# Z1HaoC/YOLO-Dual

Hardware: AMD Instinct MI355X
Metric: images/sec at 640x640 bs=16/GPU (higher is better)
Workload: dtype bf16; 1 GPU; YOLOv5-backbone (C3+SPPF) + UNet-lite SegmentHead, fwd+bwd+SGD/EMA step, 640x640, bs=16/GPU, CE+0.5*Dice, 12 classes (BASELINE configs[1]); global_batch=16, parallelism=dp1

## Files before the change

### yolo_dual_amd/csrc/spatial.hip

```cpp
#include "common.h"
#include <stdlib.h>

static inline int sgrid(long long total) {
    long long b = (total + 255) / 256;
    if (b > 256 * 16) b = 256 * 16;
    if (b < 1) b = 1;
    return (int)b;
}

template <typename T>
__global__ __launch_bounds__(256) void maxpool_fwd_kernel(const T* __restrict__ x, int ldx, T* __restrict__ y, int ldy,
                                                          uint8_t* __restrict__ idx, int N, int Hi, int Wi, int Ho, int Wo,
                                                          int Cp, int k, int s, int p) {
    constexpr int V = ET<T>::V;
    const int cpp = Cp / V;
    const long long total = (long long)N * Ho * Wo * cpp;
    for (long long i = (long long)blockIdx.x * blockDim.x + threadIdx.x; i < total; i += (long long)gridDim.x * blockDim.x) {
        int cq = (int)(i % cpp);
        long long pix = i / cpp;
        int wo = (int)(pix % Wo);
        long long t2 = pix / Wo;
        int ho = (int)(t2 % Ho);
        int n = (int)(t2 / Ho);
        float best[V];
        int bi[V];
#pragma unroll
        for (int e = 0; e < V; ++e) { best[e] = -INFINITY; bi[e] = 0; }
        bool first = true;
        for (int ky = 0; ky < k; ++ky) {
            int ih = ho * s - p + ky;
            if ((unsigned)ih >= (unsigned)Hi) continue;
            for (int kx = 0; kx < k; ++kx) {
                int iw = wo * s - p + kx;
                if ((unsigned)iw >= (unsigned)Wi) continue;
                float v[V];
                unpack16<T>(*(const uint4*)(x + ((size_t)(n * Hi + ih) * Wi + iw) * ldx + cq * V), v);
#pragma unroll
                for (int e = 0; e < V; ++e) {
                    if (first || v[e] > best[e] || v[e] != v[e]) { best[e] = v[e]; bi[e] = ky * k + kx; }
                }
                first = false;
            }
        }
        *(uint4*)(y + (size_t)pix * ldy + cq * V) = pack16<T>(best);
        if (idx) {
#pragma unroll
            for (int e = 0; e < V; ++e) idx[(size_t)pix * Cp + cq * V + e] = (uint8_t)bi[e];
        }
    }
}

template <typename T>
__global__ __launch_bounds__(256) void maxpool_bwd_kernel(const T* __restrict__ dy, int lddy, const uint8_t* __restrict__ idx,
                                                          T* __restrict__ dx, int lddx, int accumulate, int N, int Hi, int Wi,
                                                          int Ho, int Wo, int Cp, int k, int s, int p) {
    constexpr int V = ET<T>::V;
    const int cpp = Cp / V;
    const long long total = (long long)N * Hi * Wi * cpp;
    for (long long i = (long long)blockIdx.x * blockDim.x + threadIdx.x; i < total; i += (long long)gridDim.x * blockDim.x) {
        int cq = (int)(i % cpp);
        long long pix = i / cpp;
        int iw = (int)(pix % Wi);
        long long t2 = pix / Wi;
        int ih = (int)(t2 % Hi);
        int n = (int)(t2 / Hi);
        float g[V];
#pragma unroll
        for (int e = 0; e < V; ++e) g[e] = 0.f;
        if (accumulate) unpack16<T>(*(const uint4*)(dx + (size_t)pix * lddx + cq * V), g);
        for (int ky = 0; ky < k; ++ky) {
            int nh = ih + p - ky;
            if (nh < 0 || nh % s != 0) continue;
            int ho = nh / s;
            if (ho >= Ho) continue;
            for (int kx = 0; kx < k; ++kx) {
                int nw = iw + p - kx;
                if (nw < 0 || nw % s != 0) continue;
                int wo = nw / s;
                if (wo >= Wo) continue;
                size_t op = ((size_t)(n * Ho + ho) * Wo + wo);
                float d[V];
                unpack16<T>(*(const uint4*)(dy + op * lddy + cq * V), d);
                const uint8_t* ip = idx + op * Cp + cq * V;
                int code = ky * k + kx;
#pragma unroll
                for (int e = 0; e < V; ++e) g[e] += (ip[e] == code) ? d[e] : 0.f;
            }
        }
        *(uint4*)(dx + (size_t)pix * lddx + cq * V) = pack16<T>(g);
    }
}

extern "C" int ydl_maxpool_fwd(int dtype, const void* x, int ldx, void* y, int ldy, uint8_t* idx,
                               int N, int Hi, int Wi, int Ho, int Wo, int C, int k, int s, int p, void* stream) {
    const int V = dtype == YDL_F32 ? 4 : 8;
    const int Cp = round_up(C, V);
    YDL_CHECK(x && y && ldx >= Cp && ldy >= Cp && k * k <= 255, "bad arguments");
    YDL_CHECK(Ho == (Hi + 2 * p - k) / s + 1 && Wo == (Wi + 2 * p - k) / s + 1, "output size mismatch");
    hipStream_t st = (hipStream_t)stream;
    int grid = sgrid((long long)N * Ho * Wo * (Cp / V));
    if (dtype == YDL_F32) maxpool_fwd_kernel<float><<<grid, 256, 0, st>>>((const float*)x, ldx, (float*)y, ldy, idx, N, Hi, Wi, Ho, Wo, Cp, k, s, p);
    else maxpool_fwd_kernel<bf16_t><<<grid, 256, 0, st>>>((const bf16_t*)x, ldx, (bf16_t*)y, ldy, idx, N, Hi, Wi, Ho, Wo, Cp, k, s, p);
    YDL_LAUNCH_CHECK();
    return 0;
}
extern "C" int ydl_maxpool_bwd(int dtype, const void* dy, int lddy, const uint8_t* idx, void* dx, int lddx, int accumulate,
                               int N, int Hi, int Wi, int Ho, int Wo, int C, int k, int s, int p, void* stream) {
    const int V = dtype == YDL_F32 ? 4 : 8;
    const int Cp = round_up(C, V);
    YDL_CHECK(dy && dx && idx && lddy >= Cp && lddx >= Cp, "bad arguments");
    hipStream_t st = (hipStream_t)stream;
    int grid = sgrid((long long)N * Hi * Wi * (Cp / V));
    if (dtype == YDL_F32) maxpool_bwd_kernel<float><<<grid, 256, 0, st>>>((const float*)dy, lddy, idx, (float*)dx, lddx, accumulate, N, Hi, Wi, Ho, Wo, Cp, k, s, p);
    else maxpool_bwd_kernel<bf16_t><<<grid, 256, 0, st>>>((const bf16_t*)dy, lddy, idx, (bf16_t*)dx, lddx, accumulate, N, Hi, Wi, Ho, Wo, Cp, k, s, p);
    YDL_LAUNCH_CHECK();
    return 0;
}

template <int V> struct SpCodes;
template <> struct SpCodes<8> {
    typedef uint2 W;
    __device__ static __forceinline__ W pack(const int* c) {
        return make_uint2((unsigned)c[0] | ((unsigned)c[1] << 8) | ((unsigned)c[2] << 16) | ((unsigned)c[3] << 24),
                          (unsigned)c[4] | ((unsigned)c[5] << 8) | ((unsigned)c[6] << 16) | ((unsigned)c[7] << 24));
    }
    __device__ static __forceinline__ int get(const W& w, int e) { return (int)(((e < 4 ? w.x : w.y) >> ((e & 3) * 8)) & 0xffu); }
};
template <> struct SpCodes<4> {
    typedef unsigned W;
    __device__ static __forceinline__ W pack(const int* c) {
        return (unsigned)c[0] | ((unsigned)c[1] << 8) | ((unsigned)c[2] << 16) | ((unsigned)c[3] << 24);
    }
    __device__ static __forceinline__ int get(const W& w, int e) { return (int)((w >> (e * 8)) & 0xffu); }
};
#define SP_CG 2
template <typename T>
__global__ __launch_bounds__(256) void sppf_pool_fwd_kernel(const T* __restrict__ x, int ldx, T* __restrict__ y1, T* __restrict__ y2,
                                                            T* __restrict__ y3, int ldy, uint8_t* __restrict__ i1, uint8_t* __restrict__ i2,
                                                            uint8_t* __restrict__ i3, int H, int W, int Cp, int k) {
    constexpr int V = ET<T>::V;
    extern __shared__ __attribute__((aligned(16))) unsigned char sp_smem[];
    const int HW = H * W;
    const int items = HW * SP_CG;
    uint4* cur = (uint4*)sp_smem;
    uint4* rmax = cur + items;
    typedef SpCodes<V> CW;
    typename CW::W* rkx = (typename CW::W*)(rmax + items);
    const int cpp = Cp / V;
    const int n = blockIdx.y;
    const int cq0 = blockIdx.x * SP_CG;
    const int p = k / 2;
    for (int it = threadIdx.x; it < items; it += 256) {
        const int cg = it % SP_CG, pix = it / SP_CG;
        uint4 v = make_uint4(0, 0, 0, 0);
        if (cq0 + cg < cpp) v = *(const uint4*)(x + ((size_t)n * HW + pix) * ldx + (cq0 + cg) * V);
        cur[it] = v;
    }
    __syncthreads();
    T* const ys[3] = {y1, y2, y3};
    uint8_t* const is[3] = {i1, i2, i3};
#pragma unroll
    for (int st = 0; st < 3; ++st) {
        for (int it = threadIdx.x; it < items; it += 256) {
            const int cg = it % SP_CG, pix = it / SP_CG;
            const int wo = pix % W, ho = pix / W;
            float best[V];
            int bk[V];
#pragma unroll
            for (int e = 0; e < V; ++e) { best[e] = -INFINITY; bk[e] = 0; }
            bool first = true;
            for (int kx = 0; kx < k; ++kx) {
                const int iw = wo - p + kx;
                if ((unsigned)iw >= (unsigned)W) continue;
                float v[V];
                unpack16<T>(cur[(ho * W + iw) * SP_CG + cg], v);
#pragma unroll
                for (int e = 0; e < V; ++e)
                    if (first || v[e] > best[e] || v[e] != v[e]) { best[e] = v[e]; bk[e] = kx; }
                first = false;
            }
            rmax[it] = pack16<T>(best);
            rkx[it] = CW::pack(bk);
        }
        __syncthreads();
        for (int it = threadIdx.x; it < items; it += 256) {
            const int cg = it % SP_CG, pix = it / SP_CG;
            const int wo = pix % W, ho = pix / W;
            float best[V];
            int bi[V];
#pragma unroll
            for (int e = 0; e < V; ++e) { best[e] = -INFINITY; bi[e] = 0; }
            bool first = true;
            for (int ky = 0; ky < k; ++ky) {
                const int ih = ho - p + ky;
                if ((unsigned)ih >= (unsigned)H) continue;
                const int rit = (ih * W + wo) * SP_CG + cg;
                float v[V];
                unpack16<T>(rmax[rit], v);
                const typename CW::W rk = rkx[rit];
#pragma unroll
                for (int e = 0; e < V; ++e)
                    if (first || v[e] > best[e] || v[e] != v[e]) { best[e] = v[e]; bi[e] = ky * k + CW::get(rk, e); }
                first = false;
            }
            const uint4 o = pack16<T>(best);
            if (st < 2) cur[it] = o;
            if (cq0 + cg < cpp) {
                const size_t gp = (size_t)n * HW + pix;
                *(uint4*)(ys[st] + gp * ldy + (cq0 + cg) * V) = o;
                if (is[st]) *(typename CW::W*)(is[st] + gp * Cp + (cq0 + cg) * V) = CW::pack(bi);
            }
        }
        __syncthreads();
    }
}

template <typename T>
__global__ __launch_bounds__(256) void sppf_pool_bwd_kernel(const T* __restrict__ dy1, const T* __restrict__ dy2, const T* __restrict__ dy3,
                                                            int lddy, const uint8_t* __restrict__ i1, const uint8_t* __restrict__ i2,
                                                            const uint8_t* __restrict__ i3, T* __restrict__ dx, int lddx, int accumulate,
                                                            int H, int W, int Cp, int k) {
    constexpr int V = ET<T>::V;
    extern __shared__ __attribute__((aligned(16))) unsigned char sp_smem[];
    const int HW = H * W;
    uint4* plane[2] = {(uint4*)sp_smem, (uint4*)sp_smem + (size_t)HW * SP_CG};
    typedef SpCodes<V> CW;
    typename CW::W* icode = (typename CW::W*)((uint4*)sp_smem + (size_t)2 * HW * SP_CG);
    const int cpp = Cp / V;
    const int n = blockIdx.y;
    const int cq0 = blockIdx.x * SP_CG;
    const int p = k / 2;
    const int items = HW * SP_CG;
    const T* const dys[3] = {dy3, dy2, dy1};
    const uint8_t* const is[3] = {i3, i2, i1};
    for (int it = threadIdx.x; it < items; it += 256) {
        const int cg = it % SP_CG, pix = it / SP_CG;
        uint4 v = make_uint4(0, 0, 0, 0);
        if (cq0 + cg < cpp) v = *(const uint4*)(dy3 + ((size_t)n * HW + pix) * lddy + (cq0 + cg) * V);
        plane[0][it] = v;
    }
#pragma unroll
    for (int st = 0; st < 3; ++st) {
        for (int it = threadIdx.x; it < items; it += 256) {
            const int cg = it % SP_CG, pix = it / SP_CG;
            if (cq0 + cg < cpp) icode[it] = *(const typename CW::W*)(is[st] + ((size_t)n * HW + pix) * Cp + (cq0 + cg) * V);
        }
        __syncthreads();
        const uint4* src = plane[st & 1];
        uint4* dst = plane[(st + 1) & 1];
        for (int it = threadIdx.x; it < items; it += 256) {
            const int cg = it % SP_CG, pix = it / SP_CG;
            if (cq0 + cg >= cpp) continue;
            const int iw = pix % W, ih = pix / W;
            const size_t gp = (size_t)n * HW + pix;
            float g[V];
#pragma unroll
            for (int e = 0; e < V; ++e) g[e] = 0.f;
            if (st < 2) unpack16<T>(*(const uint4*)(dys[st + 1] + gp * lddy + (cq0 + cg) * V), g);
            else if (accumulate) unpack16<T>(*(const uint4*)(dx + gp * lddx + (cq0 + cg) * V), g);
            for (int ky = 0; ky < k; ++ky) {
                const int ho = ih + p - ky;
                if (ho < 0 || ho >= H) continue;
                for (int kx = 0; kx < k; ++kx) {
                    const int wo = iw + p - kx;
                    if (wo < 0 || wo >= W) continue;
                    const int oit = (ho * W + wo) * SP_CG + cg;
                    float d[V];
                    unpack16<T>(src[oit], d);
                    const typename CW::W cw = icode[oit];
                    const int code = ky * k + kx;
#pragma unroll
                    for (int e = 0; e < V; ++e) g[e] += (CW::get(cw, e) == code) ? d[e] : 0.f;
                }
            }
            const uint4 o = pack16<T>(g);
            if (st < 2) dst[it] = o;
            else *(uint4*)(dx + gp * lddx + (cq0 + cg) * V) = o;
        }
        __syncthreads();
    }
}

static inline size_t sppf_smem(int dtype, int H, int W, bool bwd) {
    const int V = dtype == YDL_F32 ? 4 : 8;
    (void)bwd;
    return (size_t)H * W * SP_CG * (2 * 16 + V);
}
extern "C" int ydl_sppf_pool_supported(int dtype, int H, int W, int C, int k) {
    if (dtype != YDL_F32 && dtype != YDL_BF16) return 0;
    if (k < 1 || k % 2 == 0 || k * k > 255 || H < 1 || W < 1 || C < 1) return 0;
    return sppf_smem(dtype, H, W, true) <= 64 * 1024 ? 1 : 0;
}
extern "C" int ydl_sppf_pool_fwd(int dtype, const void* x, int ldx, void* y1, void* y2, void* y3, int ldy,
                                 uint8_t* idx1, uint8_t* idx2, uint8_t* idx3, int N, int H, int W, int C, int k, void* stream) {
    const int V = dtype == YDL_F32 ? 4 : 8;
    const int Cp = round_up(C, V);
    YDL_CHECK(ydl_sppf_pool_supported(dtype, H, W, C, k), "plane too large for the LDS-resident form (query ydl_sppf_pool_supported)");
    YDL_CHECK(x && y1 && y2 && y3 && ldx >= Cp && ldy >= Cp && N >= 1, "bad arguments");
    YDL_CHECK((idx1 == nullptr) == (idx2 == nullptr) && (idx2 == nullptr) == (idx3 == nullptr), "the three index planes come together");
    YDL_CHECK(aligned16(x) && aligned16(y1) && aligned16(y2) && aligned16(y3) && ldx % V == 0 && ldy % V == 0, "16-byte alignment");
    hipStream_t st = (hipStream_t)stream;
    const dim3 grid((Cp / V + SP_CG - 1) / SP_CG, N);
    const size_t smem = sppf_smem(dtype, H, W, false);
    if (dtype == YDL_F32) sppf_pool_fwd_kernel<float><<<grid, 256, smem, st>>>((const float*)x, ldx, (float*)y1, (float*)y2, (float*)y3, ldy, idx1, idx2, idx3, H, W, Cp, k);
    else sppf_pool_fwd_kernel<bf16_t><<<grid, 256, smem, st>>>((const bf16_t*)x, ldx, (bf16_t*)y1, (bf16_t*)y2, (bf16_t*)y3, ldy, idx1, idx2, idx3, H, W, Cp, k);
    YDL_LAUNCH_CHECK();
    return 0;
}
extern "C" int ydl_sppf_pool_bwd(int dtype, const void* dy1, const void* dy2, const void* dy3, int lddy, const uint8_t* idx1,
                                 const uint8_t* idx2, const uint8_t* idx3, void* dx, int lddx, int accumulate,
                                 int N, int H, int W, int C, int k, void* stream) {
    const int V = dtype == YDL_F32 ? 4 : 8;
    const int Cp = round_up(C, V);
    YDL_CHECK(ydl_sppf_pool_supported(dtype, H, W, C, k), "plane too large for the LDS-resident form (query ydl_sppf_pool_supported)");
    YDL_CHECK(dy1 && dy2 && dy3 && idx1 && idx2 && idx3 && dx && lddy >= Cp && lddx >= Cp && N >= 1, "bad arguments");
    YDL_CHECK(aligned16(dy1) && aligned16(dy2) && aligned16(dy3) && aligned16(dx) && lddy % V == 0 && lddx % V == 0, "16-byte alignment");
    hipStream_t st = (hipStream_t)stream;
    const dim3 grid((Cp / V + SP_CG - 1) / SP_CG, N);
    const size_t smem = sppf_smem(dtype, H, W, true);
    if (dtype == YDL_F32) sppf_pool_bwd_kernel<float><<<grid, 256, smem, st>>>((const float*)dy1, (const float*)dy2, (const float*)dy3, lddy, idx1, idx2, idx3, (float*)dx, lddx, accumulate, H, W, Cp, k);
    else sppf_pool_bwd_kernel<bf16_t><<<grid, 256, smem, st>>>((const bf16_t*)dy1, (const bf16_t*)dy2, (const bf16_t*)dy3, lddy, idx1, idx2, idx3, (bf16_t*)dx, lddx, accumulate, H, W, Cp, k);
    YDL_LAUNCH_CHECK();
    return 0;
}

struct Lin { int i0, i1; float w0, w1; };

__device__ __forceinline__ Lin lin_src(int dst, float scale, int in, bool align) {
    Lin L;
    float src;
    if (align) {
        src = __fmul_rn(scale, (float)dst);
    } else {
        src = __fsub_rn(__fmul_rn(scale, __fadd_rn((float)dst, 0.5f)), 0.5f);
        if (src < 0.f) src = 0.f;
    }
    L.i0 = (int)src;
    if (L.i0 > in - 1) L.i0 = in - 1;
    L.i1 = L.i0 + (L.i0 < in - 1 ? 1 : 0);
    L.w1 = __fsub_rn(src, (float)L.i0);
    L.w0 = __fsub_rn(1.f, L.w1);
    return L;
}
__device__ __forceinline__ int near_src(int dst, float scale, int in) {
    int v = (int)floorf(__fmul_rn((float)dst, scale));
    return v < in - 1 ? v : in - 1;
}

template <typename T>
__global__ __launch_bounds__(256) void resize_fwd_kernel(int mode, const T* __restrict__ x, int ldx, T* __restrict__ y, int ldy,
                                                         int N, int Hi, int Wi, int Ho, int Wo, int Cp, float sh, float sw) {
    constexpr int V = ET<T>::V;
    const int cpp = Cp / V;
    const long long total = (long long)N * Ho * Wo * cpp;
    for (long long i = (long long)blockIdx.x * blockDim.x + threadIdx.x; i < total; i += (long long)gridDim.x * blockDim.x) {
        int cq = (int)(i % cpp);
        long long pix = i / cpp;
        int wo = (int)(pix % Wo);
        long long t2 = pix / Wo;
        int ho = (int)(t2 % Ho);
        int n = (int)(t2 / Ho);
        const T* xb = x + (size_t)n * Hi * Wi * ldx + cq * V;
        float o[V];
        if (mode == 0) {
            int ih = near_src(ho, sh, Hi), iw = near_src(wo, sw, Wi);
            *(uint4*)(y + (size_t)pix * ldy + cq * V) = *(const uint4*)(xb + ((size_t)ih * Wi + iw) * ldx);
            continue;
        }
        Lin lh = lin_src(ho, sh, Hi, mode == 2), lw = lin_src(wo, sw, Wi, mode == 2);
        float v00[V], v01[V], v10[V], v11[V];
        unpack16<T>(*(const uint4*)(xb + ((size_t)lh.i0 * Wi + lw.i0) * ldx), v00);
        unpack16<T>(*(const uint4*)(xb + ((size_t)lh.i0 * Wi + lw.i1) * ldx), v01);
        unpack16<T>(*(const uint4*)(xb + ((size_t)lh.i1 * Wi + lw.i0) * ldx), v10);
        unpack16<T>(*(const uint4*)(xb + ((size_t)lh.i1 * Wi + lw.i1) * ldx), v11);
#pragma unroll
        for (int e = 0; e < V; ++e)
            o[e] = lh.w0 * (lw.w0 * v00[e] + lw.w1 * v01[e]) + lh.w1 * (lw.w0 * v10[e] + lw.w1 * v11[e]);
        *(uint4*)(y + (size_t)pix * ldy + cq * V) = pack16<T>(o);
    }
}

__device__ __forceinline__ void cand_range(int i, int in, int out, float scale, int mode, int& lo, int& hi) {
    float inv = scale > 0.f ? 1.0f / scale : (float)out;
    float a = ((float)i - 1.5f) * inv - 2.f, b = ((float)i + 1.5f) * inv + 2.f;
    if (mode == 0) { a = (float)i * inv - 2.f; b = ((float)i + 1.f) * inv + 2.f; }
    lo = a < 0.f ? 0 : (int)a;
    hi = b > (float)(out - 1) ? out - 1 : (int)b;
    if (i == in - 1) hi = out - 1;
    if (i == 0) lo = 0;
}

template <typename T>
__global__ __launch_bounds__(256) void resize_bwd_kernel(int mode, const T* __restrict__ dy, int lddy, T* __restrict__ dx, int lddx,
                                                         int accumulate, int N, int Hi, int Wi, int Ho, int Wo, int Cp, float sh, float sw) {
    constexpr int V = ET<T>::V;
    const int cpp = Cp / V;
    const long long total = (long long)N * Hi * Wi * cpp;
    for (long long i = (long long)blockIdx.x * blockDim.x + threadIdx.x; i < total; i += (long long)gridDim.x * blockDim.x) {
        int cq = (int)(i % cpp);
        long long pix = i / cpp;
        int iw = (int)(pix % Wi);
        long long t2 = pix / Wi;
        int ih = (int)(t2 % Hi);
        int n = (int)(t2 / Hi);
        float g[V];
#pragma unroll
        for (int e = 0; e < V; ++e) g[e] = 0.f;
        if (accumulate) unpack16<T>(*(const uint4*)(dx + (size_t)pix * lddx + cq * V), g);
        int hlo, hhi, wlo, whi;
        cand_range(ih, Hi, Ho, sh, mode, hlo, hhi);
        cand_range(iw, Wi, Wo, sw, mode, wlo, whi);
        const T* db = dy + (size_t)n * Ho * Wo * lddy + cq * V;
        for (int ho = hlo; ho <= hhi; ++ho) {
            float wh;
            if (mode == 0) wh = near_src(ho, sh, Hi) == ih ? 1.f : 0.f;
            else { Lin l = lin_src(ho, sh, Hi, mode == 2); wh = (l.i0 == ih ? l.w0 : 0.f) + (l.i1 == ih ? l.w1 : 0.f); }
            if (wh == 0.f) continue;
            for (int wo = wlo; wo <= whi; ++wo) {
                float ww;
                if (mode == 0) ww = near_src(wo, sw, Wi) == iw ? 1.f : 0.f;
                else { Lin l = lin_src(wo, sw, Wi, mode == 2); ww = (l.i0 == iw ? l.w0 : 0.f) + (l.i1 == iw ? l.w1 : 0.f); }
                if (ww == 0.f) continue;
                float d[V];
                unpack16<T>(*(const uint4*)(db + ((size_t)ho * Wo + wo) * lddy), d);
                float wgt = wh * ww;
#pragma unroll
                for (int e = 0; e < V; ++e) g[e] += wgt * d[e];
            }
        }
        *(uint4*)(dx + (size_t)pix * lddx + cq * V) = pack16<T>(g);
    }
}

template <typename T, int S>
__global__ __launch_bounds__(256) void resize_bwd_int_kernel(const T* __restrict__ dy, int lddy, T* __restrict__ dx, int lddx, int accumulate,
                                                             int N, int Hi, int Wi, int Cp, float sh, float sw) {
    constexpr int V = ET<T>::V;
    constexpr int NC = 2 * S;
    const int Ho = Hi * S, Wo = Wi * S;
    const int cpp = Cp / V;
    const long long total = (long long)N * Hi * Wi * cpp;
    for (long long i = (long long)blockIdx.x * blockDim.x + threadIdx.x; i < total; i += (long long)gridDim.x * blockDim.x) {
        const int cq = (int)(i % cpp);
        const long long pix = i / cpp;
        const int iw = (int)(pix % Wi);
        const long long t2 = pix / Wi;
        const int ih = (int)(t2 % Hi);
        const int n = (int)(t2 / Hi);
        float g[V];
#pragma unroll
        for (int e = 0; e < V; ++e) g[e] = 0.f;
        if (accumulate) unpack16<T>(*(const uint4*)(dx + (size_t)pix * lddx + cq * V), g);
        float wwv[NC];
#pragma unroll
        for (int b = 0; b < NC; ++b) {
            const int wo = S * iw - S / 2 + b;
            float ww = 0.f;
            if ((unsigned)wo < (unsigned)Wo) { const Lin l = lin_src(wo, sw, Wi, false); ww = (l.i0 == iw ? l.w0 : 0.f) + (l.i1 == iw ? l.w1 : 0.f); }
            wwv[b] = ww;
        }
        const T* db = dy + (size_t)n * Ho * Wo * lddy + cq * V;
#pragma unroll
        for (int a = 0; a < NC; ++a) {
            const int ho = S * ih - S / 2 + a;
            if ((unsigned)ho >= (unsigned)Ho) continue;
            const Lin l = lin_src(ho, sh, Hi, false);
            const float wh = (l.i0 == ih ? l.w0 : 0.f) + (l.i1 == ih ? l.w1 : 0.f);
            if (wh == 0.f) continue;
#pragma unroll
            for (int b = 0; b < NC; ++b) {
                const int wo = S * iw - S / 2 + b;
                if (wwv[b] == 0.f) continue;
                float d[V];
                unpack16<T>(*(const uint4*)(db + ((size_t)ho * Wo + wo) * lddy), d);
                const float wgt = wh * wwv[b];
#pragma unroll
                for (int e = 0; e < V; ++e) g[e] += wgt * d[e];
            }
        }
        *(uint4*)(dx + (size_t)pix * lddx + cq * V) = pack16<T>(g);
    }
}

template <typename T, bool ACC>
__global__ __launch_bounds__(256) void resize_acc_sums_kernel(int mode, const T* __restrict__ x, int ldx, T* __restrict__ y, int ldy,
                                                              int Hi, int Wi, int Ho, int Wo, int Cp, float sh, float sw,
                                                              int nrows, float* __restrict__ sums, int sums_ld) {
    constexpr int V = ET<T>::V;
    const int cpp = Cp / V;
    const int cpb = cpp < 256 ? cpp : 256;
    const int R = 256 / cpb;
    const int cq = threadIdx.x % cpb, pl = threadIdx.x / cpb;
    const int chunk = blockIdx.y * 256 + cq;
    const bool live = pl < R && chunk < cpp;
    const int c0 = chunk * V;
    float s1[V], s2[V];
#pragma unroll
    for (int e = 0; e < V; ++e) { s1[e] = 0.f; s2[e] = 0.f; }
    if (live) {
        for (int row = blockIdx.x; row < nrows; row += gridDim.x) {
            const int n = row / Ho, ho = row - n * Ho;
            const T* xb = x + (size_t)n * Hi * Wi * ldx + c0;
            T* yrow = y + (size_t)row * Wo * ldy + c0;
            Lin lh;
            int ihn = 0;
            if (mode == 0) ihn = near_src(ho, sh, Hi);
            else lh = lin_src(ho, sh, Hi, mode == 2);
            const T* r0 = xb + (size_t)(mode == 0 ? ihn : lh.i0) * Wi * ldx;
            const T* r1 = xb + (size_t)(mode == 0 ? ihn : lh.i1) * Wi * ldx;
            for (int wo = pl; wo < Wo; wo += R) {
                float o[V], yv[V];
                if (mode == 0) {
                    unpack16<T>(*(const uint4*)(r0 + (size_t)near_src(wo, sw, Wi) * ldx), o);
                } else {
                    const Lin lw = lin_src(wo, sw, Wi, mode == 2);
                    float v00[V], v01[V], v10[V], v11[V];
                    unpack16<T>(*(const uint4*)(r0 + (size_t)lw.i0 * ldx), v00);
                    unpack16<T>(*(const uint4*)(r0 + (size_t)lw.i1 * ldx), v01);
                    unpack16<T>(*(const uint4*)(r1 + (size_t)lw.i0 * ldx), v10);
                    unpack16<T>(*(const uint4*)(r1 + (size_t)lw.i1 * ldx), v11);
#pragma unroll
                    for (int e = 0; e < V; ++e)
                        o[e] = lh.w0 * (lw.w0 * v00[e] + lw.w1 * v01[e]) + lh.w1 * (lw.w0 * v10[e] + lw.w1 * v11[e]);
                }
                T* yp = yrow + (size_t)wo * ldy;
                if constexpr (ACC) {
                    unpack16<T>(*(const uint4*)yp, yv);
#pragma unroll
                    for (int e = 0; e < V; ++e) {
                        const float v = yv[e] + o[e];
                        yv[e] = v;
                        s1[e] += v;
                        s2[e] = fmaf(v, v, s2[e]);
                    }
                    *(uint4*)yp = pack16<T>(yv);
                } else {
                    *(uint4*)yp = pack16<T>(o);
                }
            }
        }
    }
    if (!ACC || sums == nullptr) return;
    __shared__ float red[256 * 2 * 8];
#pragma unroll
    for (int e = 0; e < V; ++e) {
        red[(threadIdx.x * 2 + 0) * V + e] = live ? s1[e] : 0.f;
        red[(threadIdx.x * 2 + 1) * V + e] = live ? s2[e] : 0.f;
    }
    __syncthreads();
    if (threadIdx.x < cpb && chunk < cpp) {
        float* dst = sums + (size_t)(blockIdx.x & (YDL_BN_REPLICAS - 1)) * 2 * sums_ld;
#pragma unroll
        for (int e = 0; e < V; ++e) {
            float a = 0.f, b = 0.f;
            for (int l = 0; l < R; ++l) {
                const int tt = l * cpb + threadIdx.x;
                a += red[(tt * 2 + 0) * V + e];
                b += red[(tt * 2 + 1) * V + e];
            }
            atomicAdd(dst + c0 + e, a);
            atomicAdd(dst + sums_ld + c0 + e, b);
        }
    }
}

int g_resize_rows = 1;
int g_resize_int = 1;
static inline float axis_scale(int mode, int in, int out, float given) {
    if (mode == 2) return out > 1 ? (float)(in - 1) / (float)(out - 1) : 0.f;
    if (given > 0.f) return given;
    return (float)in / (float)out;
}

extern "C" int ydl_resize_fwd(int dtype, int mode, const void* x, int ldx, void* y, int ldy,
                              int N, int Hi, int Wi, int Ho, int Wo, int C, float scale_h, float scale_w, void* stream) {
    const int V = dtype == YDL_F32 ? 4 : 8;
    const int Cp = round_up(C, V);
    YDL_CHECK(x && y && mode >= 0 && mode <= 2 && ldx >= Cp && ldy >= Cp, "bad arguments");
    float sh = axis_scale(mode, Hi, Ho, scale_h), sw = axis_scale(mode, Wi, Wo, scale_w);
    hipStream_t st = (hipStream_t)stream;
    if (g_resize_rows && (long long)N * Ho < (1ll << 30)) {
        const int nrows = N * Ho, cpp = Cp / V;
        const dim3 grid((unsigned)(nrows < 4096 ? nrows : 4096), (unsigned)((cpp + 255) / 256));
        if (dtype == YDL_F32) resize_acc_sums_kernel<float, false><<<grid, 256, 0, st>>>(mode, (const float*)x, ldx, (float*)y, ldy, Hi, Wi, Ho, Wo, Cp, sh, sw, nrows, nullptr, 0);
        else resize_acc_sums_kernel<bf16_t, false><<<grid, 256, 0, st>>>(mode, (const bf16_t*)x, ldx, (bf16_t*)y, ldy, Hi, Wi, Ho, Wo, Cp, sh, sw, nrows, nullptr, 0);
        YDL_LAUNCH_CHECK();
        return 0;
    }
    int grid = sgrid((long long)N * Ho * Wo * (Cp / V));
    if (dtype == YDL_F32) resize_fwd_kernel<float><<<grid, 256, 0, st>>>(mode, (const float*)x, ldx, (float*)y, ldy, N, Hi, Wi, Ho, Wo, Cp, sh, sw);
    else resize_fwd_kernel<bf16_t><<<grid, 256, 0, st>>>(mode, (const bf16_t*)x, ldx, (bf16_t*)y, ldy, N, Hi, Wi, Ho, Wo, Cp, sh, sw);
    YDL_LAUNCH_CHECK();
    return 0;
}
extern "C" int ydl_resize_acc_sums(int dtype, int mode, const void* x, int ldx, void* y, int ldy, int N, int Hi, int Wi, int Ho, int Wo,
                                   int C, float scale_h, float scale_w, float* sums, int sums_ld, void* stream) {
    const int V = dtype == YDL_F32 ? 4 : 8;
    const int Cp = round_up(C, V);
    YDL_CHECK(x && y && mode >= 0 && mode <= 2 && ldx >= Cp && ldy >= Cp && N >= 1, "bad arguments");
    YDL_CHECK(aligned16(x) && aligned16(y) && ldx % V == 0 && ldy % V == 0, "16-byte alignment");
    YDL_CHECK(sums == nullptr || sums_ld >= Cp, "statistics rows shorter than the padded channel count");
    const float sh = axis_scale(mode, Hi, Ho, scale_h), sw = axis_scale(mode, Wi, Wo, scale_w);
    hipStream_t st = (hipStream_t)stream;
    const int cpp = Cp / V;
    YDL_CHECK((long long)N * Ho < (1ll << 30), "too many output rows");
    const int nrows = N * Ho;
    const dim3 grid((unsigned)(nrows < 4096 ? nrows : 4096), (unsigned)((cpp + 255) / 256));
    if (dtype == YDL_F32) resize_acc_sums_kernel<float, true><<<grid, 256, 0, st>>>(mode, (const float*)x, ldx, (float*)y, ldy, Hi, Wi, Ho, Wo, Cp, sh, sw, nrows, sums, sums_ld);
    else resize_acc_sums_kernel<bf16_t, true><<<grid, 256, 0, st>>>(mode, (const bf16_t*)x, ldx, (bf16_t*)y, ldy, Hi, Wi, Ho, Wo, Cp, sh, sw, nrows, sums, sums_ld);
    YDL_LAUNCH_CHECK();
    return 0;
}
extern "C" int ydl_resize_bwd(int dtype, int mode, const void* dy, int lddy, void* dx, int lddx, int accumulate,
                              int N, int Hi, int Wi, int Ho, int Wo, int C, float scale_h, float scale_w, void* stream) {
    const int V = dtype == YDL_F32 ? 4 : 8;
    const int Cp = round_up(C, V);
    YDL_CHECK(dy && dx && mode >= 0 && mode <= 2 && lddy >= Cp && lddx >= Cp, "bad arguments");
    float sh = axis_scale(mode, Hi, Ho, scale_h), sw = axis_scale(mode, Wi, Wo, scale_w);
    hipStream_t st = (hipStream_t)stream;
    int grid = sgrid((long long)N * Hi * Wi * (Cp / V));
    const int Sq = (Wi > 0 && Wo % Wi == 0) ? Wo / Wi : 0;
    if (g_resize_int && mode == 1 && (Sq == 2 || Sq == 4) && Ho == Hi * Sq && sh == 1.f / (float)Sq && sw == 1.f / (float)Sq) {
        const int S = Sq;
        if (dtype == YDL_F32) {
// ... 443 lines not shown
```

Baseline: 2567 images/sec.

## Specialize SPPF LDS pooling kernels on kernel size and adaptive channel grouping

Templates the SPPF fused max-pool forward and backward kernels on channel-group width and kernel size. Channel groups per block and thread count are chosen from the plane size, up to 512 threads, and the window loops are fully unrolled with branch-free neighbor indexing. The backward kernel now preloads all three index planes into LDS once with a single barrier, instead of reloading and syncing each stage. The aim is less index arithmetic, fewer barriers and better occupancy on the small 20x20 SPPF plane. The cost is more template instantiations, higher LDS use in backward, and a new H*W<=819 cap on the supported shapes.

```diff
diff --git a/yolo_dual_amd/csrc/spatial.hip b/yolo_dual_amd/csrc/spatial.hip
--- a/yolo_dual_amd/csrc/spatial.hip
+++ b/yolo_dual_amd/csrc/spatial.hip
@@ -125,6 +125,7 @@
                           (unsigned)c[4] | ((unsigned)c[5] << 8) | ((unsigned)c[6] << 16) | ((unsigned)c[7] << 24));
     }
     __device__ static __forceinline__ int get(const W& w, int e) { return (int)(((e < 4 ? w.x : w.y) >> ((e & 3) * 8)) & 0xffu); }
+    __device__ static __forceinline__ W add(const W& w, int c) { return make_uint2(w.x + (unsigned)c * 0x01010101u, w.y + (unsigned)c * 0x01010101u); }
 };
 template <> struct SpCodes<4> {
     typedef unsigned W;
@@ -132,26 +133,35 @@
         return (unsigned)c[0] | ((unsigned)c[1] << 8) | ((unsigned)c[2] << 16) | ((unsigned)c[3] << 24);
     }
     __device__ static __forceinline__ int get(const W& w, int e) { return (int)((w >> (e * 8)) & 0xffu); }
+    __device__ static __forceinline__ W add(const W& w, int c) { return w + (unsigned)c * 0x01010101u; }
 };
-#define SP_CG 2
-template <typename T>
-__global__ __launch_bounds__(256) void sppf_pool_fwd_kernel(const T* __restrict__ x, int ldx, T* __restrict__ y1, T* __restrict__ y2,
-                                                            T* __restrict__ y3, int ldy, uint8_t* __restrict__ i1, uint8_t* __restrict__ i2,
-                                                            uint8_t* __restrict__ i3, int H, int W, int Cp, int k) {
+#define SP_MAX_THREADS 512
+static inline int sppf_cg(int HW) { return HW >= 256 ? 1 : HW >= 128 ? 2 : 4; }
+static inline int sppf_threads(int items) {
+    const int trips = (items + SP_MAX_THREADS - 1) / SP_MAX_THREADS;
+    return round_up((items + trips - 1) / trips, 64);
+}
+template <typename T, int CG, int K>
+__global__ __launch_bounds__(SP_MAX_THREADS) void sppf_pool_fwd_kernel(const T* __restrict__ x, int ldx, T* __restrict__ y1, T* __restrict__ y2,
+                                                                       T* __restrict__ y3, int ldy, uint8_t* __restrict__ i1,
+                                                                       uint8_t* __restrict__ i2, uint8_t* __restrict__ i3, int H, int W,
+                                                                       int Cp, int kr) {
     constexpr int V = ET<T>::V;
     extern __shared__ __attribute__((aligned(16))) unsigned char sp_smem[];
+    const int k = K ? K : kr;
+    const int nt = blockDim.x;
     const int HW = H * W;
-    const int items = HW * SP_CG;
+    const int items = HW * CG;
     uint4* cur = (uint4*)sp_smem;
     uint4* rmax = cur + items;
     typedef SpCodes<V> CW;
     typename CW::W* rkx = (typename CW::W*)(rmax + items);
     const int cpp = Cp / V;
     const int n = blockIdx.y;
-    const int cq0 = blockIdx.x * SP_CG;
+    const int cq0 = blockIdx.x * CG;
     const int p = k / 2;
-    for (int it = threadIdx.x; it < items; it += 256) {
-        const int cg = it % SP_CG, pix = it / SP_CG;
+    for (int it = threadIdx.x; it < items; it += nt) {
+        const int cg = it % CG, pix = it / CG;
         uint4 v = make_uint4(0, 0, 0, 0);
         if (cq0 + cg < cpp) v = *(const uint4*)(x + ((size_t)n * HW + pix) * ldx + (cq0 + cg) * V);
         cur[it] = v;
@@ -161,47 +171,46 @@
     uint8_t* const is[3] = {i1, i2, i3};
 #pragma unroll
     for (int st = 0; st < 3; ++st) {
-        for (int it = threadIdx.x; it < items; it += 256) {
-            const int cg = it % SP_CG, pix = it / SP_CG;
-            const int wo = pix % W, ho = pix / W;
+        for (int it = threadIdx.x; it < items; it += nt) {
+            const int pix = it / CG;
+            const int wo = pix % W;
             float best[V];
             int bk[V];
-#pragma unroll
-            for (int e = 0; e < V; ++e) { best[e] = -INFINITY; bk[e] = 0; }
-            bool first = true;
+            const int kx0 = p > wo ? p - wo : 0;
+#pragma unroll
+            for (int e = 0; e < V; ++e) { best[e] = -INFINITY; bk[e] = kx0; }
+#pragma unroll
             for (int kx = 0; kx < k; ++kx) {
-                const int iw = wo - p + kx;
-                if ((unsigned)iw >= (unsigned)W) continue;
+                const bool ok = (unsigned)(wo - p + kx) < (unsigned)W;
                 float v[V];
-                unpack16<T>(cur[(ho * W + iw) * SP_CG + cg], v);
+                unpack16<T>(cur[ok ? it + (kx - p) * CG : it], v);
 #pragma unroll
                 for (int e = 0; e < V; ++e)
-                    if (first || v[e] > best[e] || v[e] != v[e]) { best[e] = v[e]; bk[e] = kx; }
-                first = false;
+                    if (ok && (v[e] > best[e] || v[e] != v[e])) { best[e] = v[e]; bk[e] = kx; }
             }
             rmax[it] = pack16<T>(best);
             rkx[it] = CW::pack(bk);
         }
         __syncthreads();
-        for (int it = threadIdx.x; it < items; it += 256) {
-            const int cg = it % SP_CG, pix = it / SP_CG;
-            const int wo = pix % W, ho = pix / W;
+        for (int it = threadIdx.x; it < items; it += nt) {
+            const int cg = it % CG, pix = it / CG;
+            const int ho = pix / W;
             float best[V];
             int bi[V];
+            const int ky0 = p > ho ? p - ho : 0;
 #pragma unroll
             for (int e = 0; e < V; ++e) { best[e] = -INFINITY; bi[e] = 0; }
-            bool first = true;
+#pragma unroll
             for (int ky = 0; ky < k; ++ky) {
-                const int ih = ho - p + ky;
-                if ((unsigned)ih >= (unsigned)H) continue;
-                const int rit = (ih * W + wo) * SP_CG + cg;
+                const bool ok = (unsigned)(ho - p + ky) < (unsigned)H;
+                const bool frc = ky == ky0;
+                const int rit = ok ? it + (ky - p) * W * CG : it;
                 float v[V];
                 unpack16<T>(rmax[rit], v);
-                const typename CW::W rk = rkx[rit];
+                const typename CW::W rc = CW::add(rkx[rit], ky * k);
 #pragma unroll
                 for (int e = 0; e < V; ++e)
-                    if (first || v[e] > best[e] || v[e] != v[e]) { best[e] = v[e]; bi[e] = ky * k + CW::get(rk, e); }
-                first = false;
+                    if (ok && (frc || v[e] > best[e] || v[e] != v[e])) { best[e] = v[e]; bi[e] = CW::get(rc, e); }
             }
             const uint4 o = pack16<T>(best);
             if (st < 2) cur[it] = o;
@@ -215,41 +224,49 @@
     }
 }
 
-template <typename T>
-__global__ __launch_bounds__(256) void sppf_pool_bwd_kernel(const T* __restrict__ dy1, const T* __restrict__ dy2, const T* __restrict__ dy3,
-                                                            int lddy, const uint8_t* __restrict__ i1, const uint8_t* __restrict__ i2,
-                                                            const uint8_t* __restrict__ i3, T* __restrict__ dx, int lddx, int accumulate,
-                                                            int H, int W, int Cp, int k) {
+template <typename T, int CG, int K>
+__global__ __launch_bounds__(SP_MAX_THREADS) void sppf_pool_bwd_kernel(const T* __restrict__ dy1, const T* __restrict__ dy2,
+                                                                       const T* __restrict__ dy3, int lddy, const uint8_t* __restrict__ i1,
+                                                                       const uint8_t* __restrict__ i2, const uint8_t* __restrict__ i3,
+                                                                       T* __restrict__ dx, int lddx, int accumulate, int H, int W, int Cp,
+                                                                       int kr) {
     constexpr int V = ET<T>::V;
     extern __shared__ __attribute__((aligned(16))) unsigned char sp_smem[];
+    const int k = K ? K : kr;
+    const int nt = blockDim.x;
     const int HW = H * W;
-    uint4* plane[2] = {(uint4*)sp_smem, (uint4*)sp_smem + (size_t)HW * SP_CG};
+    const int items = HW * CG;
+    uint4* plane[2] = {(uint4*)sp_smem, (uint4*)sp_smem + items};
     typedef SpCodes<V> CW;
-    typename CW::W* icode = (typename CW::W*)((uint4*)sp_smem + (size_t)2 * HW * SP_CG);
+    typename CW::W* icode = (typename CW::W*)((uint4*)sp_smem + (size_t)2 * items);
     const int cpp = Cp / V;
     const int n = blockIdx.y;
-    const int cq0 = blockIdx.x * SP_CG;
+    const int cq0 = blockIdx.x * CG;
     const int p = k / 2;
-    const int items = HW * SP_CG;
     const T* const dys[3] = {dy3, dy2, dy1};
     const uint8_t* const is[3] = {i3, i2, i1};
-    for (int it = threadIdx.x; it < items; it += 256) {
-        const int cg = it % SP_CG, pix = it / SP_CG;
+    for (int it = threadIdx.x; it < items; it += nt) {
+        const int cg = it % CG, pix = it / CG;
         uint4 v = make_uint4(0, 0, 0, 0);
-        if (cq0 + cg < cpp) v = *(const uint4*)(dy3 + ((size_t)n * HW + pix) * lddy + (cq0 + cg) * V);
+        typename CW::W c[3] = {};
+        if (cq0 + cg < cpp) {
+            const size_t gp = (size_t)n * HW + pix;
+            v = *(const uint4*)(dy3 + gp * lddy + (cq0 + cg) * V);
+#pragma unroll
+            for (int st = 0; st < 3; ++st) c[st] = *(const typename CW::W*)(is[st] + gp * Cp + (cq0 + cg) * V);
+        }
         plane[0][it] = v;
-    }
+#pragma unroll
+        for (int st = 0; st < 3; ++st) icode[st * items + it] = c[st];
+    }
+    __syncthreads();
 #pragma unroll
     for (int st = 0; st < 3; ++st) {
-        for (int it = threadIdx.x; it < items; it += 256) {
-            const int cg = it % SP_CG, pix = it / SP_CG;
-            if (cq0 + cg < cpp) icode[it] = *(const typename CW::W*)(is[st] + ((size_t)n * HW + pix) * Cp + (cq0 + cg) * V);
-        }
-        __syncthreads();
         const uint4* src = plane[st & 1];
         uint4* dst = plane[(st + 1) & 1];
-        for (int it = threadIdx.x; it < items; it += 256) {
-            const int cg = it % SP_CG, pix = it / SP_CG;
+        const typename CW::W* code_st = icode + st * items;
+        for (int it = threadIdx.x; it < items; it += nt) {
+            const int cg = it % CG, pix = it / CG;
             if (cq0 + cg >= cpp) continue;
             const int iw = pix % W, ih = pix / W;
             const size_t gp = (size_t)n * HW + pix;
@@ -258,19 +275,20 @@
             for (int e = 0; e < V; ++e) g[e] = 0.f;
             if (st < 2) unpack16<T>(*(const uint4*)(dys[st + 1] + gp * lddy + (cq0 + cg) * V), g);
             else if (accumulate) unpack16<T>(*(const uint4*)(dx + gp * lddx + (cq0 + cg) * V), g);
+#pragma unroll 1
             for (int ky = 0; ky < k; ++ky) {
-                const int ho = ih + p - ky;
-                if (ho < 0 || ho >= H) continue;
+                const bool oky = (unsigned)(ih + p - ky) < (unsigned)H;
+#pragma unroll
                 for (int kx = 0; kx < k; ++kx) {
-                    const int wo = iw + p - kx;
-                    if (wo < 0 || wo >= W) continue;
-                    const int oit = (ho * W + wo) * SP_CG + cg;
+                    const bool ok = oky && (unsigned)(iw + p - kx) < (unsigned)W;
+                    const int oit = ok ? it + ((p - ky) * W + (p - kx)) * CG : it;
                     float d[V];
                     unpack16<T>(src[oit], d);
-                    const typename CW::W cw = icode[oit];
+                    const typename CW::W cw = code_st[oit];
                     const int code = ky * k + kx;
-#pragma unroll
-                    for (int e = 0; e < V; ++e) g[e] += (CW::get(cw, e) == code) ? d[e] : 0.f;
+                    const float miss = ok ? 0.f : -0.f;
+#pragma unroll
+                    for (int e = 0; e < V; ++e) g[e] += (ok && CW::get(cw, e) == code) ? d[e] : miss;
                 }
             }
             const uint4 o = pack16<T>(g);
@@ -281,29 +299,43 @@
     }
 }
 
-static inline size_t sppf_smem(int dtype, int H, int W, bool bwd) {
-    const int V = dtype == YDL_F32 ? 4 : 8;
-    (void)bwd;
-    return (size_t)H * W * SP_CG * (2 * 16 + V);
+static inline size_t sppf_smem(int dtype, int H, int W, int cg, bool bwd) {
+    const int V = dtype == YDL_F32 ? 4 : 8;
+    return (size_t)H * W * cg * (2 * 16 + (bwd ? 3 : 1) * V);
 }
 extern "C" int ydl_sppf_pool_supported(int dtype, int H, int W, int C, int k) {
     if (dtype != YDL_F32 && dtype != YDL_BF16) return 0;
     if (k < 1 || k % 2 == 0 || k * k > 255 || H < 1 || W < 1 || C < 1) return 0;
-    return sppf_smem(dtype, H, W, true) <= 64 * 1024 ? 1 : 0;
-}
+    if ((long long)H * W > 819) return 0;
+    return sppf_smem(dtype, H, W, sppf_cg(H * W), true) <= 64 * 1024 ? 1 : 0;
+}
+#define SPPF_DISPATCH_K(KERNEL, T, CGV, ...)                                                              \
+    do {                                                                                                  \
+        if (k == 5) KERNEL<T, CGV, 5><<<grid, threads, smem, st>>>(__VA_ARGS__);                         \
+        else if (k == 3) KERNEL<T, CGV, 3><<<grid, threads, smem, st>>>(__VA_ARGS__);                    \
+        else KERNEL<T, CGV, 0><<<grid, threads, smem, st>>>(__VA_ARGS__);                                \
+    } while (0)
+#define SPPF_DISPATCH(KERNEL, T, ...)                                                                     \
+    do {                                                                                                  \
+        if (cg == 1) SPPF_DISPATCH_K(KERNEL, T, 1, __VA_ARGS__);                                          \
+        else if (cg == 2) SPPF_DISPATCH_K(KERNEL, T, 2, __VA_ARGS__);                                     \
+        else SPPF_DISPATCH_K(KERNEL, T, 4, __VA_ARGS__);                                                  \
+    } while (0)
 extern "C" int ydl_sppf_pool_fwd(int dtype, const void* x, int ldx, void* y1, void* y2, void* y3, int ldy,
                                  uint8_t* idx1, uint8_t* idx2, uint8_t* idx3, int N, int H, int W, int C, int k, void* stream) {
     const int V = dtype == YDL_F32 ? 4 : 8;
     const int Cp = round_up(C, V);
     YDL_CHECK(ydl_sppf_pool_supported(dtype, H, W, C, k), "plane too large for the LDS-resident form (query ydl_sppf_pool_supported)");
-    YDL_CHECK(x && y1 && y2 && y3 && ldx >= Cp && ldy >= Cp && N >= 1, "bad arguments");
+    YDL_CHECK(x && y1 && y2 && y3 && ldx >= Cp && ldy >= Cp && N >= 1 && N <= 65535, "bad arguments");
     YDL_CHECK((idx1 == nullptr) == (idx2 == nullptr) && (idx2 == nullptr) == (idx3 == nullptr), "the three index planes come together");
     YDL_CHECK(aligned16(x) && aligned16(y1) && aligned16(y2) && aligned16(y3) && ldx % V == 0 && ldy % V == 0, "16-byte alignment");
     hipStream_t st = (hipStream_t)stream;
-    const dim3 grid((Cp / V + SP_CG - 1) / SP_CG, N);
-    const size_t smem = sppf_smem(dtype, H, W, false);
-    if (dtype == YDL_F32) sppf_pool_fwd_kernel<float><<<grid, 256, smem, st>>>((const float*)x, ldx, (float*)y1, (float*)y2, (float*)y3, ldy, idx1, idx2, idx3, H, W, Cp, k);
-    else sppf_pool_fwd_kernel<bf16_t><<<grid, 256, smem, st>>>((const bf16_t*)x, ldx, (bf16_t*)y1, (bf16_t*)y2, (bf16_t*)y3, ldy, idx1, idx2, idx3, H, W, Cp, k);
+    const int cg = sppf_cg(H * W);
+    const int threads = sppf_threads(H * W * cg);
+    const dim3 grid((Cp / V + cg - 1) / cg, N);
+    const size_t smem = sppf_smem(dtype, H, W, cg, false);
+    if (dtype == YDL_F32) SPPF_DISPATCH(sppf_pool_fwd_kernel, float, (const float*)x, ldx, (float*)y1, (float*)y2, (float*)y3, ldy, idx1, idx2, idx3, H, W, Cp, k);
+    else SPPF_DISPATCH(sppf_pool_fwd_kernel, bf16_t, (const bf16_t*)x, ldx, (bf16_t*)y1, (bf16_t*)y2, (bf16_t*)y3, ldy, idx1, idx2, idx3, H, W, Cp, k);
     YDL_LAUNCH_CHECK();
     return 0;
 }
@@ -313,13 +345,15 @@
     const int V = dtype == YDL_F32 ? 4 : 8;
     const int Cp = round_up(C, V);
     YDL_CHECK(ydl_sppf_pool_supported(dtype, H, W, C, k), "plane too large for the LDS-resident form (query ydl_sppf_pool_supported)");
-    YDL_CHECK(dy1 && dy2 && dy3 && idx1 && idx2 && idx3 && dx && lddy >= Cp && lddx >= Cp && N >= 1, "bad arguments");
+    YDL_CHECK(dy1 && dy2 && dy3 && idx1 && idx2 && idx3 && dx && lddy >= Cp && lddx >= Cp && N >= 1 && N <= 65535, "bad arguments");
     YDL_CHECK(aligned16(dy1) && aligned16(dy2) && aligned16(dy3) && aligned16(dx) && lddy % V == 0 && lddx % V == 0, "16-byte alignment");
     hipStream_t st = (hipStream_t)stream;
-    const dim3 grid((Cp / V + SP_CG - 1) / SP_CG, N);
-    const size_t smem = sppf_smem(dtype, H, W, true);
-    if (dtype == YDL_F32) sppf_pool_bwd_kernel<float><<<grid, 256, smem, st>>>((const float*)dy1, (const float*)dy2, (const float*)dy3, lddy, idx1, idx2, idx3, (float*)dx, lddx, accumulate, H, W, Cp, k);
-    else sppf_pool_bwd_kernel<bf16_t><<<grid, 256, smem, st>>>((const bf16_t*)dy1, (const bf16_t*)dy2, (const bf16_t*)dy3, lddy, idx1, idx2, idx3, (bf16_t*)dx, lddx, accumulate, H, W, Cp, k);
+    const int cg = sppf_cg(H * W);
+    const int threads = sppf_threads(H * W * cg);
+    const dim3 grid((Cp / V + cg - 1) / cg, N);
+    const size_t smem = sppf_smem(dtype, H, W, cg, true);
+    if (dtype == YDL_F32) SPPF_DISPATCH(sppf_pool_bwd_kernel, float, (const float*)dy1, (const float*)dy2, (const float*)dy3, lddy, idx1, idx2, idx3, (float*)dx, lddx, accumulate, H, W, Cp, k);
+    else SPPF_DISPATCH(sppf_pool_bwd_kernel, bf16_t, (const bf16_t*)dy1, (const bf16_t*)dy2, (const bf16_t*)dy3, lddy, idx1, idx2, idx3, (bf16_t*)dx, lddx, accumulate, H, W, Cp, k);
     YDL_LAUNCH_CHECK();
     return 0;
 }
```

Measured after the change: 2556 images/sec. Within noise of the previous version (-0.4%).
